# shanpenghui/ExtractORB

Measured on AMD Instinct MI355X. Metric: frames/sec (ORB extract, 640x480x8-level x1000 feat), higher is better.
Workload: dtype u8; 1 GPU; mono640: 640x480 mono stream, 8 levels, 1000 features, synthetic noise frames; variant=noise, nfeatures=1000, nlevels=8, handles_per_gpu=1, parallelism=frames sharded 512/GPU

## Files before the change

### extractorb_amd/csrc/k_pyramid.hip

```cpp
#include <hip/hip_runtime.h>
#include <stdint.h>

#include "orbx_device.hpp"

namespace orbx {

__device__ __forceinline__ int reflect101(int p, int n) {
    p = p < 0 ? -p : p;
    return p >= n ? 2 * (n - 1) - p : p;
}

constexpr int kPyrRows = kResizeTileRows / 4;
constexpr int kTileCols = 64;
constexpr int kTileRowGroups = 4;
constexpr int kTileRows = kPyrRows * kTileRowGroups;

static __host__ __device__ inline int rowDwords(const LevelGeom& g) { return (kPadL - kEdge + g.w + 2 * kEdge + 3) / 4; }

struct SrcView {
    const uint8_t* p;
    long long frame;
    int stride;
    int readableCols;
    int aligned;
};

__device__ __forceinline__ unsigned mulHi24(unsigned a, unsigned b) {
    unsigned r;
    asm("v_mul_hi_u32_u24 %0, %1, %2" : "=v"(r) : "v"(a), "v"(b));
    return r;
}
__device__ __forceinline__ unsigned pkLshr2(unsigned a) {
    unsigned r;
    asm("v_pk_lshrrev_b16 %0, %2, %1" : "=v"(r) : "v"(a), "s"(0x00020002u));
    return r;
}
typedef unsigned short u16x2 __attribute__((ext_vector_type(2)));

template <bool PACKED>
__device__ __forceinline__ void resizeTile(const SrcView& sv, const LevelGeom& d, const ResizeX* __restrict__ xt, const QuadRec* __restrict__ xq,
                                           const ResizeX* __restrict__ yt, const TileFoot ft, uint8_t* __restrict__ pyr,
                                           int tileX, int tileY, int f, uint8_t* tile, int ldsStride) {
    const int tid = threadIdx.x, col = tid & (kTileCols - 1), rgrp = tid / kTileCols;
    const int nd = rowDwords(d), wB = d.w + 2 * kEdge;
    const int dw = tileX * kTileCols + col;
    const bool valid = dw < nd;
    const int bc0 = 4 * (valid ? dw : nd - 1);
    const int fx0 = ft.fx0, fy0 = ft.fy0, nDw = ft.nDw, nRows = ft.nRows;
    const uint8_t* sp = sv.p + (long long)f * sv.frame;

    int c0[4], c1[4], a0[4], a1[4];
    uint4 q0{}, q1{};
    int qlo = 0;
    if constexpr (PACKED) {
        const uint4* qr = (const uint4*)(xq + (valid ? dw : nd - 1));
        q0 = qr[0]; q1 = qr[1];
        qlo = ((const int*)qr)[9] - fx0;
    } else {
#pragma unroll
        for (int j = 0; j < 4; j++) {
            int bx = bc0 + j - (kPadL - kEdge);
            bx = bx < 0 ? 0 : (bx > wB - 1 ? wB - 1 : bx);
            const ResizeX cx = xt[reflect101(bx - kEdge, d.w)];
            c0[j] = cx.sx0 - fx0; c1[j] = cx.sx1 - fx0; a0[j] = cx.a0; a1[j] = cx.a1;
        }
    }
    __shared__ __align__(16) RowRec ycoef[kTileRows];
    RowRec myY{};
    if (tid < kTileRows) myY = makeRowRec(yt[reflect101(min(tileY * kTileRows + tid, d.pyrRows - 1) - kEdge, d.h)]);

    {
        constexpr int kStageRows = 12;
        const int c = tid & 127, rsub = tid >> 7;
        for (int cc = c; cc < nDw; cc += 128) {
            const bool whole = sv.aligned && fx0 + 4 * cc + 3 < sv.readableCols;
            const int colOff = fx0 + 4 * cc;
            for (int rb = rsub; rb < nRows; rb += 2 * kStageRows) {
                unsigned w[kStageRows];
#pragma unroll
                for (int k = 0; k < kStageRows; k++) {
                    const int r = min(rb + 2 * k, nRows - 1);
                    const uint8_t* q = sp + (__mul24(fy0 + r, sv.stride) + colOff);
                    if (whole) {
                        w[k] = *(const unsigned*)q;
                    } else {
                        w[k] = 0;
#pragma unroll
                        for (int b = 0; b < 4; b++)
                            if (fx0 + 4 * cc + b < sv.readableCols) w[k] |= (unsigned)q[b] << (8 * b);
                    }
                }
#pragma unroll
                for (int k = 0; k < kStageRows; k++)
                    if (rb + 2 * k < nRows) *(unsigned*)(tile + (rb + 2 * k) * ldsStride + 4 * cc) = w[k];
            }
        }
    }
    if (tid < kTileRows) ycoef[tid] = myY;
    __syncthreads();
    const int by0 = tileY * kTileRows + rgrp * kPyrRows;
    const RowRec* cy = ycoef + rgrp * kPyrRows;
    uint8_t* dst = pyr + d.pyrOff + (long long)f * d.pyrFrameBytes + (long long)by0 * d.pyrStride + bc0;
    if constexpr (PACKED) {
        const int base = qlo & ~3;
        const unsigned sh = (unsigned)(qlo & 3);
        const unsigned sel[4] = {q0.x, q0.y, q0.z, q0.w};
        const u16x2 wt[4] = {__builtin_bit_cast(u16x2, q1.x), __builtin_bit_cast(u16x2, q1.y), __builtin_bit_cast(u16x2, q1.z), __builtin_bit_cast(u16x2, q1.w)};
        auto hrow = [&](int srow, unsigned (&h)[4]) {
            const unsigned* rp = (const unsigned*)(tile + __mul24(srow - fy0, ldsStride) + base);
            const unsigned p0 = rp[0], p1 = rp[1], p2 = rp[2];
            const unsigned P0 = __builtin_amdgcn_alignbyte(p1, p0, sh), P1 = __builtin_amdgcn_alignbyte(p2, p1, sh);
#pragma unroll
            for (int j = 0; j < 4; j++)
                h[j] = __builtin_amdgcn_udot2(__builtin_bit_cast(u16x2, __builtin_amdgcn_perm(P1, P0, sel[j])), wt[j], 0u, false) & ~15u;
        };
        unsigned HA[4] = {0, 0, 0, 0}, HB[4] = {0, 0, 0, 0};
        int haveA = -(1 << 20), haveB = -(1 << 20);
#pragma unroll
        for (int r = 0; r < kPyrRows; r++) {
            const RowRec rr = cy[r];
            const int sA = __builtin_amdgcn_readfirstlane(rr.sA), sB = __builtin_amdgcn_readfirstlane(rr.sB);
            if (sA != haveA) { hrow(sA, HA); haveA = sA; }
            if (sB != haveB) { hrow(sB, HB); haveB = sB; }
            unsigned t[4];
#pragma unroll
            for (int j = 0; j < 4; j++) t[j] = mulHi24(rr.bA, HA[j]) + mulHi24(rr.bB, HB[j]) + 2u;
            const unsigned u01 = pkLshr2(t[0] | (t[1] << 16)), u23 = pkLshr2(t[2] | (t[3] << 16));
            if (valid && by0 + r < d.pyrRows) *(unsigned*)(dst + r * d.pyrStride) = __builtin_amdgcn_perm(u23, u01, 0x06040200u);
        }
    } else {
#pragma unroll 2
    for (int r = 0; r < kPyrRows; r++) {
        const uint8_t* r0 = tile + __mul24(cy[r].sA - fy0, ldsStride);
        const uint8_t* r1 = tile + __mul24(cy[r].sB - fy0, ldsStride);
        const int b0 = (int)(cy[r].bA >> 12), b1 = (int)(cy[r].bB >> 12);
        unsigned o = 0;
#pragma unroll
        for (int j = 0; j < 4; j++) {
            const int h0 = __mul24(r0[c0[j]], a0[j]) + __mul24(r0[c1[j]], a1[j]);
            const int h1 = __mul24(r1[c0[j]], a0[j]) + __mul24(r1[c1[j]], a1[j]);
            const int v = ((__mul24(b0, h0 >> 4) >> 16) + (__mul24(b1, h1 >> 4) >> 16) + 2) >> 2;
            o |= (unsigned)v << (8 * j);
        }
        if (valid && by0 + r < d.pyrRows) *(unsigned*)(dst + r * d.pyrStride) = o;
    }
    }
}

__device__ __forceinline__ void copyTile(const SrcView& sv, const LevelGeom& g0, uint8_t* __restrict__ pyr, int tileX,
                                         int tileY, int f) {
    const int tid = threadIdx.x, col = tid & (kTileCols - 1), rgrp = tid / kTileCols;
    const int dw = tileX * kTileCols + col;
    if (dw >= rowDwords(g0)) return;
    const int wB = g0.w + 2 * kEdge, bc0 = 4 * dw;
    const int x0 = bc0 - kPadL;
    const bool inner = sv.aligned && x0 >= 0 && x0 + 3 < g0.w;
    int sx[4];
#pragma unroll
    for (int j = 0; j < 4; j++) {
        int bx = bc0 + j - (kPadL - kEdge);
        bx = bx < 0 ? 0 : (bx > wB - 1 ? wB - 1 : bx);
        sx[j] = reflect101(bx - kEdge, g0.w);
    }
    const uint8_t* sp = sv.p + (long long)f * sv.frame;
    const int by0 = tileY * kTileRows + rgrp * kPyrRows;
    unsigned out[kPyrRows];
#pragma unroll
    for (int r = 0; r < kPyrRows; r++) {
        const uint8_t* row = sp + __mul24(reflect101(min(by0 + r, g0.pyrRows - 1) - kEdge, g0.h), sv.stride);
        if (inner) out[r] = *(const unsigned*)(row + x0);
        else out[r] = (unsigned)row[sx[0]] | ((unsigned)row[sx[1]] << 8) | ((unsigned)row[sx[2]] << 16) | ((unsigned)row[sx[3]] << 24);
    }
    uint8_t* dst = pyr + g0.pyrOff + (long long)f * g0.pyrFrameBytes + (long long)by0 * g0.pyrStride + bc0;
#pragma unroll
    for (int r = 0; r < kPyrRows; r++)
        if (by0 + r < g0.pyrRows) *(unsigned*)(dst + r * g0.pyrStride) = out[r];
}

template <bool PACKED>
__global__ __launch_bounds__(256) void k_pyr_first(SrcView img, LevelGeom g0, LevelGeom g1, int tilesX0, int nTiles0,
                                                    int tilesX1, const ResizeX* __restrict__ xt, const QuadRec* __restrict__ xq, const ResizeX* __restrict__ yt,
                                                    const TileFoot* __restrict__ foot, uint8_t* __restrict__ pyr, int ldsStride, int f0, int nFrames) {
    extern __shared__ __align__(16) uint8_t tile[];
    int t, fr;
    if (!xcdChunkFrame(nFrames, t, fr)) return;
    if (t < nTiles0) {
        const int tileY = t / tilesX0;
        copyTile(img, g0, pyr, t - tileY * tilesX0, tileY, f0 + fr);
    } else {
        t -= nTiles0;
        const int tileY = t / tilesX1;
        resizeTile<PACKED>(img, g1, xt, xq, yt, foot[t], pyr, t - tileY * tilesX1, tileY, f0 + fr, tile, ldsStride);
    }
}

template <bool PACKED>
__global__ __launch_bounds__(256) void k_resize(LevelGeom s, LevelGeom d, int tilesX, const ResizeX* __restrict__ xt, const QuadRec* __restrict__ xq,
                                                 const ResizeX* __restrict__ yt, const TileFoot* __restrict__ foot,
                                                 uint8_t* __restrict__ pyr, int ldsStride, int f0, int nFrames) {
    extern __shared__ __align__(16) uint8_t tile[];
    SrcView sv;
    sv.p = pyr + s.pyrOff + (long long)kEdge * s.pyrStride + kPadL;
    sv.stride = s.pyrStride; sv.frame = s.pyrFrameBytes; sv.readableCols = s.w + kEdge; sv.aligned = 1;
    int t, fr;
    if (!xcdChunkFrame(nFrames, t, fr)) return;
    const int tileY = t / tilesX;
    resizeTile<PACKED>(sv, d, xt, xq, yt, foot[t], pyr, t - tileY * tilesX, tileY, f0 + fr, tile, ldsStride);
}

#ifdef ORBX_CHAIN_STAMPS
__device__ unsigned long long g_chainStamps[32];
#ifndef ORBX_CHAIN_STAMP_T
#define ORBX_CHAIN_STAMP_T 0
#endif
#define CSTAMP(i) do { if (tid == 0 && t == ORBX_CHAIN_STAMP_T) g_chainStamps[i] = __builtin_amdgcn_s_memrealtime(); } while (0)
extern "C" int orbx_debug_chain_stamps(unsigned long long* out32) { return (int)hipMemcpyFromSymbol(out32, HIP_SYMBOL(g_chainStamps), sizeof(unsigned long long) * 32); }
__device__ unsigned long long g_chainSpans[3 * 2048];
extern "C" int orbx_debug_chain_spans(unsigned long long* out) { return (int)hipMemcpyFromSymbol(out, HIP_SYMBOL(g_chainSpans), sizeof(g_chainSpans)); }
#define CSPAN_BEGIN do { if (tid == 0 && t < 2048) g_chainSpans[3 * t] = __builtin_amdgcn_s_memrealtime(); } while (0)
#define CSPAN_END(lvl) do { if (tid == 0 && t < 2048) { g_chainSpans[3 * t + 1] = __builtin_amdgcn_s_memrealtime(); g_chainSpans[3 * t + 2] = (unsigned long long)(lvl); } } while (0)
#else
#define CSTAMP(i) do {} while (0)
#define CSPAN_BEGIN do {} while (0)
#define CSPAN_END(lvl) do {} while (0)
#endif

template <int T>
__device__ __forceinline__ void chainStep(const uint8_t* S, uint8_t* D, const ChainRegion rs, const ChainRegion rd, const ChainDeal dl, const ResizeX* qrs, const ResizeX* cys,
                                          const int ss, const int ds, const int tid) {
    static_assert(T == 256 || T == 512, "PyrColumn::deal holds the dealing for 256 and 512 deriving threads");
    const int nq = (rd.w + 3) >> 2, nb = dl.nb, blk = (int)(((unsigned)tid * dl.recip) >> 20), x4 = 4 * (tid - blk * nq);
    const int per = dl.per, yb = blk * per, ye = min(yb + per, (int)rd.h);
    if (blk < nb && yb < ye) {
        u16x2 wt[4];
        unsigned sel[4];
        const uint4* qr = (const uint4*)((const QuadRec*)qrs + (x4 >> 2));
        const uint4 q0 = qr[0], q1 = qr[1];
        const unsigned bs = ((const unsigned*)qr)[8];
        sel[0] = q0.x; sel[1] = q0.y; sel[2] = q0.z; sel[3] = q0.w;
        wt[0] = __builtin_bit_cast(u16x2, q1.x); wt[1] = __builtin_bit_cast(u16x2, q1.y); wt[2] = __builtin_bit_cast(u16x2, q1.z); wt[3] = __builtin_bit_cast(u16x2, q1.w);
        const int base = (int)(bs & 0xffffu);
        const unsigned sh = bs >> 16;
        auto hrow = [&](int srow, unsigned (&h)[4]) {
            const unsigned* rp = (const unsigned*)(S + __mul24(srow - rs.y0, ss) + base);
            const unsigned p0 = rp[0], p1 = rp[1], p2 = rp[2];
            const unsigned P0 = __builtin_amdgcn_alignbyte(p1, p0, sh), P1 = __builtin_amdgcn_alignbyte(p2, p1, sh);
#pragma unroll
            for (int k = 0; k < 4; k++)
                h[k] = __builtin_amdgcn_udot2(__builtin_bit_cast(u16x2, __builtin_amdgcn_perm(P1, P0, sel[k])), wt[k], 0u, false) & ~15u;
        };
        unsigned HA[4] = {0, 0, 0, 0}, HB[4] = {0, 0, 0, 0};
        int haveA = -(1 << 20), haveB = -(1 << 20);
        const RowRec* rrs = (const RowRec*)cys;
        for (int y = yb; y < ye; y++) {
            const RowRec rr = rrs[y];
            if (rr.sA != haveA) { hrow(rr.sA, HA); haveA = rr.sA; }
            if (rr.sB != haveB) { hrow(rr.sB, HB); haveB = rr.sB; }
            unsigned t[4];
#pragma unroll
            for (int k = 0; k < 4; k++) t[k] = mulHi24(rr.bA, HA[k]) + mulHi24(rr.bB, HB[k]) + 2u;
            const unsigned u01 = pkLshr2(t[0] | (t[1] << 16)), u23 = pkLshr2(t[2] | (t[3] << 16));
            *(unsigned*)(D + y * ds + x4) = __builtin_amdgcn_perm(u23, u01, 0x06040200u);
        }
    }
}

template <bool PACKED, int T, int TD>
__global__ __launch_bounds__(T) void k_pyr_cols(SrcView img, const PyrColumn* __restrict__ cols, const ColLevels* __restrict__ lvp, int nlevels,
                                                            const ResizeX* __restrict__ colCoef, int coefSlot,
                                                            uint8_t* __restrict__ pyr, int bufEvenBytes, int f0, int nFrames) {
    static_assert(TD <= T && TD % 64 == 0 && (T - TD) % 64 == 0, "roles are whole waves");
    extern __shared__ __align__(16) uint8_t lds[];
    __shared__ __align__(16) ResizeX coef[kChainCoefMax];
    struct LevelOut { ColOwn own; int w, h, stride; long long off; };
    __shared__ LevelOut outOf[kMaxLevels];
    int t, fr;
    if (!xcdChunkFrame(nFrames, t, fr)) return;
    const int f = f0 + fr, tid = threadIdx.x;
    const PyrColumn& pc = cols[t];
    const ColLevels& lv = *lvp;
    const int top = nlevels - 1;
    LevelOut myOut{};
    if (tid < nlevels) myOut = LevelOut{pc.own[tid], lv.w[tid], lv.h[tid], lv.pyrStride[tid], lv.pyrOff[tid] + (long long)f * lv.pyrFrameBytes[tid]};
    CSTAMP(0);
    CSPAN_BEGIN;
    auto bufOf = [&](int j) { return lds + ((j & 1) ? bufEvenBytes : 0); };
    constexpr int kStatic = 8;
    ChainRegion rj[kStatic + 1];
#pragma unroll
    for (int j = 0; j <= kStatic; j++) rj[j] = pc.region[j];
    {
        const ChainRegion r = rj[0];
        const int nDw = r.w >> 2, total = nDw * r.h;
        const uint8_t* src = img.p + (long long)f * img.frame + (long long)r.y0 * img.stride + r.x0;
        unsigned* dst = (unsigned*)bufOf(0);
        constexpr int kLoads = (kChainMaxH0 * kChainMaxW / 4 + T - 1) / T;
        const float inv = __frcp_rn((float)nDw);
        unsigned w[kLoads];
#pragma unroll
        for (int i = 0; i < kLoads; i++) {
            w[i] = 0;
            if (i * T < total) {
            const int idx = min(tid + i * T, total - 1);
            const int row = (int)(((float)idx + 0.5f) * inv), c = idx - row * nDw;
            const uint8_t* q = src + ((unsigned)__mul24(row, img.stride) + 4u * (unsigned)c);
            const int x = r.x0 + 4 * c;
            if (img.aligned && x >= 0 && x + 3 < img.readableCols) w[i] = *(const unsigned*)q;
            else {
#pragma unroll
                for (int b = 0; b < 4; b++) w[i] |= (unsigned)q[reflect101(x + b, img.readableCols) - x] << (8 * b);
            }
            }
        }
        constexpr int kPerThread = (kChainCoefMax + T - 1) / T;
        const int nCoef = pc.nCoef;
        const ResizeX* mine = colCoef + (size_t)t * (size_t)coefSlot;
        ResizeX cv[kPerThread];
#pragma unroll
        for (int k = 0; k < kPerThread; k++) cv[k] = tid + k * T < nCoef ? mine[tid + k * T] : ResizeX{0, 0, 0, 0};
#pragma unroll
        for (int k = 0; k < kPerThread; k++)
            if (tid + k * T < nCoef) coef[tid + k * T] = cv[k];
        if (tid < nlevels) outOf[tid] = myOut;
#pragma unroll
        for (int i = 0; i < kLoads; i++)
            if (tid + i * T < total) dst[tid + i * T] = w[i];
    }
    __syncthreads();
    CSTAMP(1);
    int off = 0;
    auto doLevel = [&](const int j, const ChainRegion rs, const ChainRegion rd) {
        const int ss = (rs.w + 3) & ~3;
        const uint8_t* S = bufOf(j);
        constexpr int TW = TD < T ? T - TD : T;
        if (j < top) {
            const ResizeX* cxs = coef + off;
            const int nqUnits = 6 * ((rd.w + 3) >> 2);
            if (tid < TD) chainStep<TD>(S, bufOf(j + 1), rs, rd, pc.deal[TD == 512][j + 1 < kMaxLevels ? j + 1 : j], cxs, cxs + nqUnits, ss, (rd.w + 3) & ~3, tid);
            off += nqUnits + 2 * rd.h;
        }
        const bool everyone = TD == T || j == top;
        const int wtid = everyone ? tid : tid - TD, wstep = everyone ? T : TW;
        if (wtid >= 0) {
        const LevelOut lo = outOf[j];
        const ColOwn own = lo.own;
        const int w = lo.w, h = lo.h, wB = w + 2 * kEdge;
        uint8_t* out = pyr + lo.off;
        const int stride = lo.stride, nrows = own.r1 - own.r0;
        const int fa = max((int)own.dw0, kPadL / 4), fb = max(fa, min((int)own.dw1, kPadL / 4 + (w >> 2)));
        if (fb > fa && (fb - fa) * nrows <= 2 * wstep) {
            const int ndw = fb - fa, total = ndw * nrows;
            const float inv = __frcp_rn((float)ndw);
            for (int i = wtid; i < total; i += wstep) {
                const int rr = (int)(((float)i + 0.5f) * inv), dw = fa + (i - rr * ndw), row = own.r0 + rr;
                const uint8_t* srow = S + __mul24(reflect101(row - kEdge, h) - rs.y0, ss) - rs.x0;
                *(unsigned*)(out + (long long)row * stride + 4 * dw) = *(const unsigned*)(srow + (4 * dw - kPadL));
            }
        } else if (fb > fa) {
            const int ndw = fb - fa;
            const float rdw = __frcp_rn((float)ndw);
            const int ngrp = max((int)(((float)wstep + 0.5f) * rdw), 1);
            const int per = (int)(((float)(nrows + ngrp - 1) + 0.5f) * __frcp_rn((float)ngrp));
            const int grp = (int)(((float)wtid + 0.5f) * rdw), c = wtid - grp * ndw;
            if (wtid >= 0 && grp < ngrp) {
                const int rA = own.r0 + grp * per, rB = min(rA + per, (int)own.r1);
                const uint8_t* scol = S + (4 * (fa + c) - kPadL - rs.x0);
                uint8_t* ocol = out + 4 * (fa + c);
                auto run = [&](const int r0, const int r1, const int src0, const int sstep) {
                    const uint8_t* sp = scol + __mul24(src0 - rs.y0, ss);
                    uint8_t* op = ocol + (long long)r0 * stride;
                    for (int row = r0; row < r1; row++, op += stride, sp += sstep) *(unsigned*)op = *(const unsigned*)sp;
                };
                const int t1 = min(rB, kEdge), m0 = max(rA, kEdge), m1 = min(rB, kEdge + h), b0 = max(rA, kEdge + h);
                if (rA < t1) run(rA, t1, kEdge - rA, -ss);
                if (m0 < m1) run(m0, m1, m0 - kEdge, ss);
                if (b0 < rB) run(b0, rB, 2 * (h - 1) - (b0 - kEdge), -ss);
            }
        }
        const int nL = fa - own.dw0, nO = nL + (own.dw1 - fb);
        if (nO > 0) {
            const int total = nO * nrows;
            const float inv = __frcp_rn((float)nO);
            for (int i = wtid; i < total; i += wstep) {
                const int rr = (int)(((float)i + 0.5f) * inv), jj = i - rr * nO, dw = jj < nL ? own.dw0 + jj : fb + (jj - nL), row = own.r0 + rr;
                const uint8_t* srow = S + __mul24(reflect101(row - kEdge, h) - rs.y0, ss) - rs.x0;
                const int bc0 = 4 * dw;
                unsigned o = 0;
#pragma unroll
                for (int k = 0; k < 4; k++) {
                    int bx = bc0 + k - (kPadL - kEdge);
                    bx = bx < 0 ? 0 : (bx > wB - 1 ? wB - 1 : bx);
                    o |= (unsigned)srow[reflect101(bx - kEdge, w)] << (8 * k);
                }
                *(unsigned*)(out + (long long)row * stride + bc0) = o;
            }
        }
        }
        __syncthreads();
        CSTAMP(j + 2);
    };
#pragma unroll
    for (int j = 0; j < kStatic; j++)
        if (j <= top) doLevel(j, rj[j], rj[j + 1]);
    for (int j = kStatic; j <= top; j++) doLevel(j, pc.region[j], pc.region[j + 1 < kMaxLevels ? j + 1 : j]);
    CSPAN_END(0);
}

void launchPyrCols(hipStream_t st, const uint8_t* img, long long stride, long long frameStride, int imgW, const PyrColumn* cols, int nCols,
                   const ColLevels* lv, int nlevels, const ResizeX* colCoef, int coefSlot, uint8_t* pyr, int ldsBytes, int bufEvenBytes,
                   bool packed, int shape, int f0, int B) {
    SrcView sv;
    sv.p = img; sv.stride = (int)stride; sv.frame = frameStride; sv.readableCols = imgW;
    sv.aligned = (((uintptr_t)img | (uintptr_t)stride | (uintptr_t)frameStride) & 3) == 0;
#define ORBX_COLS_LAUNCH(P, T, TD) hipLaunchKernelGGL((k_pyr_cols<P, T, TD>), xcdGrid(nCols, B), dim3(T), (size_t)ldsBytes, st, sv, cols, lv, nlevels, colCoef, coefSlot, \
                                                  pyr, bufEvenBytes, f0, B)
    (void)packed;
    if (shape == 6) ORBX_COLS_LAUNCH(true, 1024, 512);
    else if (shape == 4) ORBX_COLS_LAUNCH(true, 768, 256);
    else ORBX_COLS_LAUNCH(true, 512, 256);
#undef ORBX_COLS_LAUNCH
}

void launchPyrFirst(hipStream_t st, const uint8_t* img, long long stride, long long frameStride, const LevelGeom& g0,
                    const LevelGeom* g1, int tilesX0, int tilesY0, int tilesX1, int tilesY1, const ResizeX* xt, const QuadRec* xq,
                    const ResizeX* yt, const TileFoot* foot, uint8_t* pyr, int ldsStride, int ldsRows, bool packed, int f0, int B) {
    SrcView sv;
    sv.p = img; sv.stride = (int)stride; sv.frame = frameStride; sv.readableCols = g0.w;
    sv.aligned = (((uintptr_t)img | (uintptr_t)stride | (uintptr_t)frameStride) & 3) == 0;
    const int n0 = tilesX0 * tilesY0, n1 = g1 ? tilesX1 * tilesY1 : 0;
    if (packed) hipLaunchKernelGGL(k_pyr_first<true>, xcdGrid(n0 + n1, B), dim3(256), (size_t)ldsStride * ldsRows + 16, st, sv, g0,
                                   g1 ? *g1 : g0, tilesX0, n0, g1 ? tilesX1 : 1, xt, xq, yt, foot, pyr, ldsStride, f0, B);
    else hipLaunchKernelGGL(k_pyr_first<false>, xcdGrid(n0 + n1, B), dim3(256), (size_t)ldsStride * ldsRows + 16, st, sv, g0,
                            g1 ? *g1 : g0, tilesX0, n0, g1 ? tilesX1 : 1, xt, xq, yt, foot, pyr, ldsStride, f0, B);
}
void launchResize(hipStream_t st, const LevelGeom& s, const LevelGeom& d, int tilesX, int tilesY, const ResizeX* xt, const QuadRec* xq,
                  const ResizeX* yt, const TileFoot* foot, uint8_t* pyr, int ldsStride, int ldsRows, bool packed, int f0, int B) {
    if (packed) hipLaunchKernelGGL(k_resize<true>, xcdGrid(tilesX * tilesY, B), dim3(256), (size_t)ldsStride * ldsRows + 16, st, s, d,
                                   tilesX, xt, xq, yt, foot, pyr, ldsStride, f0, B);
    else hipLaunchKernelGGL(k_resize<false>, xcdGrid(tilesX * tilesY, B), dim3(256), (size_t)ldsStride * ldsRows + 16, st, s, d,
                            tilesX, xt, xq, yt, foot, pyr, ldsStride, f0, B);
}

}
```

Measured before the change: 322,400 frames/s.

## Restructure pyramid source load into plain/edge passes and permute-based border fill

Splits the level-0 tile load into a plain pass of aligned dword loads, with a precomputed per-lane row walk instead of per-element division, and a separate edge pass that precomputes the reflected byte offsets and prefetches two trips ahead. Coefficients are copied as uint2 and the row base is made wave-uniform with readfirstlane. The border-fill loop now precomputes the per-column reflect/clamp byte selectors once per lane. It then shares them across the wave via ds_bpermute and assembles each output dword with a byte perm from two LDS dwords, instead of four scattered byte reads. This adds code complexity and assumes the selectors fit in a window of two dwords and that nO fits within 64 lanes.

```diff
diff --git a/extractorb_amd/csrc/k_pyr_load_deal.hpp b/extractorb_amd/csrc/k_pyr_load_deal.hpp
--- /dev/null
+++ b/extractorb_amd/csrc/k_pyr_load_deal.hpp
@@ -0,0 +1,69 @@
+#pragma once
+#include "orbx_device.hpp"
+
+namespace orbx {
+
+ORBX_HD inline float pyrLoadRcp(int b) {
+#if defined(__HIP_DEVICE_COMPILE__)
+    return __builtin_amdgcn_rcpf((float)b);
+#else
+    return 1.0f / (float)b;
+#endif
+}
+ORBX_HD inline int pyrLoadQuot(int a, float rcpB) { return (int)(((float)a + 0.5f) * rcpB); }
+
+ORBX_HD inline int pyrLoadPlainCols(int x0, int nDw, int readableCols, int aligned) {
+    const int n = aligned ? (readableCols - x0) >> 2 : 0;
+    return n < 0 ? 0 : (n > nDw ? nDw : n);
+}
+
+struct PyrLoadPass { int c0, n, ngrp; float rcpN; };
+ORBX_HD inline PyrLoadPass makePyrLoadPass(int c0, int n, int T) {
+    PyrLoadPass p;
+    p.c0 = c0; p.n = n;
+    p.rcpN = pyrLoadRcp(n > 0 ? n : 1);
+    p.ngrp = T / (n > 0 ? n : 1);
+    return p;
+}
+ORBX_HD inline bool pyrLoadHasTrip(const PyrLoadPass& p, int k, int h) { return p.n > 0 && k * p.ngrp < h; }
+struct PyrLoadLane { int grp, c, g; };
+ORBX_HD inline PyrLoadLane pyrLoadLane(const PyrLoadPass& p, int tid) {
+    PyrLoadLane l;
+    l.grp = pyrLoadQuot(tid, p.rcpN);
+    l.c = p.c0 + (tid - l.grp * p.n);
+    l.g = l.grp < p.ngrp ? l.grp : 1 << 20;
+    return l;
+}
+ORBX_HD inline bool pyrLoadOwns(const PyrLoadPass& p, const PyrLoadLane& l, int k, int h) { return l.g < h - k * p.ngrp; }
+ORBX_HD inline int pyrLoadOpaque(int v) {
+#if defined(__HIP_DEVICE_COMPILE__)
+    asm("" : "+s"(v));
+#endif
+    return v;
+}
+struct PyrLoadWalk { unsigned own0, last, lds0; int step, ldsStep; };
+ORBX_HD inline PyrLoadWalk pyrLoadWalk(const PyrLoadPass& p, const PyrLoadLane& l, int h, int stride, unsigned colBytes, int nDw) {
+    PyrLoadWalk w;
+    w.own0 = (unsigned)(l.grp * stride) + colBytes;
+    w.last = (unsigned)((h - 1) * stride) + colBytes;
+    w.lds0 = (unsigned)(l.grp * nDw + l.c);
+    w.step = pyrLoadOpaque(p.ngrp * stride);
+    w.ldsStep = pyrLoadOpaque(p.ngrp * nDw);
+    return w;
+}
+ORBX_HD inline unsigned pyrLoadOffset(const PyrLoadWalk& w, int k) {
+    const unsigned own = w.own0 + (unsigned)(k * w.step);
+    return own < w.last ? own : w.last;
+}
+ORBX_HD inline unsigned pyrLoadLdsIndex(const PyrLoadWalk& w, int k) { return w.lds0 + (unsigned)(k * w.ldsStep); }
+
+constexpr int pyrLoadTripBound(int T) {
+    int worst = 0;
+    for (int n = 1; n <= kChainMaxW / 4; n++) {
+        const int h = kChainMaxW * kChainMaxH0 / 4 / n, ngrp = T / n, trips = (h + ngrp - 1) / ngrp;
+        if (trips > worst) worst = trips;
+    }
+    return worst;
+}
+
+}
diff --git a/extractorb_amd/csrc/k_pyramid.hip b/extractorb_amd/csrc/k_pyramid.hip
--- a/extractorb_amd/csrc/k_pyramid.hip
+++ b/extractorb_amd/csrc/k_pyramid.hip
@@ -2,12 +2,17 @@
 #include <stdint.h>
 
 #include "orbx_device.hpp"
+#include "k_pyr_load_deal.hpp"
 
 namespace orbx {
 
 __device__ __forceinline__ int reflect101(int p, int n) {
     p = p < 0 ? -p : p;
     return p >= n ? 2 * (n - 1) - p : p;
+}
+
+__device__ __forceinline__ long long uniform64(long long v) {
+    return (long long)((unsigned long long)(unsigned)__builtin_amdgcn_readfirstlane((int)(v >> 32)) << 32 | (unsigned)__builtin_amdgcn_readfirstlane((int)v));
 }
 
 constexpr int kPyrRows = kResizeTileRows / 4;
@@ -291,40 +296,59 @@
     for (int j = 0; j <= kStatic; j++) rj[j] = pc.region[j];
     {
         const ChainRegion r = rj[0];
-        const int nDw = r.w >> 2, total = nDw * r.h;
-        const uint8_t* src = img.p + (long long)f * img.frame + (long long)r.y0 * img.stride + r.x0;
+        const int nDw = r.w >> 2, h = r.h;
+        const uint8_t* rowBase = img.p + uniform64((long long)f * img.frame + (long long)r.y0 * img.stride);
         unsigned* dst = (unsigned*)bufOf(0);
-        constexpr int kLoads = (kChainMaxH0 * kChainMaxW / 4 + T - 1) / T;
-        const float inv = __frcp_rn((float)nDw);
+        constexpr int kLoads = pyrLoadTripBound(T);
+        static_assert(kLoads <= 16, "the plain pass keeps one register per trip");
+        constexpr int kEdgeAhead = 2;
+        const int nP = pyrLoadPlainCols(r.x0, nDw, img.readableCols, img.aligned);
+        const PyrLoadPass pp = makePyrLoadPass(0, nP, T), pe = makePyrLoadPass(nP, nDw - nP, T);
+        const PyrLoadLane lp = pyrLoadLane(pp, tid), le = pyrLoadLane(pe, tid);
+        const PyrLoadWalk wp = pyrLoadWalk(pp, lp, h, img.stride, (unsigned)(r.x0 + 4 * lp.c), nDw), we = pyrLoadWalk(pe, le, h, img.stride, 0u, nDw);
+        unsigned xb[4];
+#pragma unroll
+        for (int b = 0; b < 4; b++) xb[b] = (unsigned)reflect101(r.x0 + 4 * le.c + b, img.readableCols);
         unsigned w[kLoads];
 #pragma unroll
         for (int i = 0; i < kLoads; i++) {
             w[i] = 0;
-            if (i * T < total) {
-            const int idx = min(tid + i * T, total - 1);
-            const int row = (int)(((float)idx + 0.5f) * inv), c = idx - row * nDw;
-            const uint8_t* q = src + ((unsigned)__mul24(row, img.stride) + 4u * (unsigned)c);
-            const int x = r.x0 + 4 * c;
-            if (img.aligned && x >= 0 && x + 3 < img.readableCols) w[i] = *(const unsigned*)q;
-            else {
-#pragma unroll
-                for (int b = 0; b < 4; b++) w[i] |= (unsigned)q[reflect101(x + b, img.readableCols) - x] << (8 * b);
-            }
-            }
-        }
+            if (pyrLoadHasTrip(pp, i, h))
+                w[i] = *(const unsigned*)(rowBase + pyrLoadOffset(wp, i));
+        }
+        auto edgeLoad = [&](const int i, unsigned (&e)[4]) {
+            const unsigned o = pyrLoadOffset(we, i);
+#pragma unroll
+            for (int b = 0; b < 4; b++) e[b] = rowBase[o + xb[b]];
+        };
+        auto edgeStore = [&](const int i, const unsigned (&e)[4]) {
+            if (pyrLoadOwns(pe, le, i, h)) dst[pyrLoadLdsIndex(we, i)] = e[0] | e[1] << 8 | e[2] << 16 | e[3] << 24;
+        };
+        unsigned ea[kEdgeAhead][4] = {};
+#pragma unroll
+        for (int i = 0; i < kEdgeAhead; i++)
+            if (pyrLoadHasTrip(pe, i, h)) edgeLoad(i, ea[i]);
         constexpr int kPerThread = (kChainCoefMax + T - 1) / T;
         const int nCoef = pc.nCoef;
         const ResizeX* mine = colCoef + (size_t)t * (size_t)coefSlot;
-        ResizeX cv[kPerThread];
-#pragma unroll
-        for (int k = 0; k < kPerThread; k++) cv[k] = tid + k * T < nCoef ? mine[tid + k * T] : ResizeX{0, 0, 0, 0};
+        uint2 cv[kPerThread];
+#pragma unroll
+        for (int k = 0; k < kPerThread; k++) cv[k] = tid + k * T < nCoef ? ((const uint2*)mine)[tid + k * T] : uint2{0u, 0u};
 #pragma unroll
         for (int k = 0; k < kPerThread; k++)
-            if (tid + k * T < nCoef) coef[tid + k * T] = cv[k];
+            if (tid + k * T < nCoef) ((uint2*)coef)[tid + k * T] = cv[k];
         if (tid < nlevels) outOf[tid] = myOut;
 #pragma unroll
         for (int i = 0; i < kLoads; i++)
-            if (tid + i * T < total) dst[tid + i * T] = w[i];
+            if (pyrLoadHasTrip(pp, i, h) && pyrLoadOwns(pp, lp, i, h)) dst[pyrLoadLdsIndex(wp, i)] = w[i];
+#pragma unroll
+        for (int i = 0; i < kEdgeAhead; i++)
+            if (pyrLoadHasTrip(pe, i, h)) edgeStore(i, ea[i]);
+        for (int i = kEdgeAhead; pyrLoadHasTrip(pe, i, h); i++) {
+            unsigned e[4];
+            edgeLoad(i, e);
+            edgeStore(i, e);
+        }
     }
     __syncthreads();
     CSTAMP(1);
@@ -381,18 +405,24 @@
         if (nO > 0) {
             const int total = nO * nrows;
             const float inv = __frcp_rn((float)nO);
-            for (int i = wtid; i < total; i += wstep) {
-                const int rr = (int)(((float)i + 0.5f) * inv), jj = i - rr * nO, dw = jj < nL ? own.dw0 + jj : fb + (jj - nL), row = own.r0 + rr;
-                const uint8_t* srow = S + __mul24(reflect101(row - kEdge, h) - rs.y0, ss) - rs.x0;
-                const int bc0 = 4 * dw;
-                unsigned o = 0;
-#pragma unroll
-                for (int k = 0; k < 4; k++) {
-                    int bx = bc0 + k - (kPadL - kEdge);
-                    bx = bx < 0 ? 0 : (bx > wB - 1 ? wB - 1 : bx);
-                    o |= (unsigned)srow[reflect101(bx - kEdge, w)] << (8 * k);
-                }
-                *(unsigned*)(out + (long long)row * stride + bc0) = o;
+            const int lane = tid & 63, tj = min(lane, nO - 1), tdw = tj < nL ? own.dw0 + tj : fb + (tj - nL);
+            int xs[4], lo = 1 << 20;
+#pragma unroll
+            for (int k = 0; k < 4; k++) {
+                int bx = 4 * tdw + k - (kPadL - kEdge);
+                bx = bx < 0 ? 0 : (bx > wB - 1 ? wB - 1 : bx);
+                xs[k] = reflect101(bx - kEdge, w) - rs.x0;
+                lo = min(lo, xs[k]);
+            }
+            const int win = lo & ~3;
+            const int recWin = win | (tdw << 8), recSel = (xs[0] - win) | (xs[1] - win) << 8 | (xs[2] - win) << 16 | (xs[3] - win) << 24;
+            for (int i0 = wtid - lane; i0 < total; i0 += wstep) {
+                const int i = min(i0 + lane, total - 1);
+                const int rr = (int)(((float)i + 0.5f) * inv), jj = i - rr * nO, row = own.r0 + rr;
+                const int cw = __builtin_amdgcn_ds_bpermute(jj << 2, recWin), cs = __builtin_amdgcn_ds_bpermute(jj << 2, recSel);
+                const unsigned* sp = (const unsigned*)(S + __mul24(reflect101(row - kEdge, h) - rs.y0, ss) + (cw & 255));
+                const unsigned o = __builtin_amdgcn_perm(sp[1], sp[0], (unsigned)cs);
+                if (i0 + lane < total) *(unsigned*)(out + (long long)row * stride + 4 * (cw >> 8)) = o;
             }
         }
         }
```

Result: no change. 325,000 frames/s, median of 6 (+0.8%).
